# ethz-tb/orcAI

Hardware: AMD Instinct MI355X
Metric: audio_seconds_per_s (higher is better)
Workload: dtype f32; 1 GPU; orcai-V1 predict, 1 h synthetic recording @48 kHz, 1833 snippets; parallelism=independent recordings x1

## Files before the change

### include/orcai_hip.h

```cpp
#ifndef ORCAI_HIP_H
#define ORCAI_HIP_H

#include <stddef.h>
#include <stdint.h>

#ifdef __cplusplus
extern "C" {
#endif

#define ORCAI_E_BADARG (-1)
#define ORCAI_E_UNSUPPORTED (-2)

const char* orcai_version(void);


size_t orcai_frontend_workspace_bytes(void);

int orcai_frontend_reset(void* workspace, void* stream);

int orcai_pcm_decode(const void* frames, int64_t n_frames, int channels, int channel, int format, float* out, void* stream);

int orcai_pcm_decode_planar(const void* frames, int64_t n_frames, int channels, int format, float* out, int64_t stride, void* stream);

int orcai_resample_polyphase(const float* x, int64_t n_in, float* out, int64_t n_out, int L, int M, const float* table, int ntaps, void* stream);
// ... 107 lines not shown

int orcai_sepconv_route(int half, int Cin, int Cout, int H, int W, int out_layout, int extras);

int orcai_entry_windows(int windows_per_wave);

int orcai_entry_tile(int waves);

int orcai_conv0_bn_relu(const float* in, int64_t snippet_stride, int B, int H, int W, int ksize, const float* w, const float* scale,
                        const float* shift, float* out, void* stream);

int orcai_conv0_sepconv(const float* in, int64_t snippet_stride, int B, int H, int W, const float* w0, const float* scale0, const float* shift0,
                        const float* dw, const float* pw, const float* scale, const float* shift, int Cout, int relu_out, float* out, float* prev_sub,
                        void* stream);

int orcai_sepconv_bn(const float* in, int B, int Cin, int H, int W, int ksize, int relu_in, const float* dw, const float* pw, const float* scale,
                     const float* shift, int Cout, int relu_out, int out_layout, float* out, void* stream);

int orcai_pool_res_add(const float* s, const float* prev, int B, int C, int Cp, int H, int W, int ksize, const float* wr, const float* br,
                       float* out, int xpooled, void* stream);
int orcai_pool_res_add_scatter(const float* s, const float* prev, int B, int C, int Cp, int H, int W, int ksize, const float* wr, const float* br,
                               float* out, int xpooled, int Hd, int nsnip, int period, int base, int img_step, int r_lo, int r_hi, int keep_lo,
                               int keep_hi, void* stream);
#define ORCAI_ROW_FAMILIES 4
typedef struct {
  float* out;
  int Hd, period, offset, count, keep_lo, keep_hi;
} orcai_row_family;
int orcai_pool_res_add_scatter_families(const float* s, const float* prev, int B, int C, int Cp, int H, int W, int ksize, const float* wr,
                                        const float* br, int xpooled, int base, int img_step, int r_lo, int r_hi, const orcai_row_family* fams,
                                        int nfam, void* stream);
int orcai_sepconv_pool_res(const float* in, const float* prev, int B, int Cin, int C, int Cp, int H, int W, int ksize, int relu_in, const float* dw, const float* pw,
                           const float* scale, const float* shift, int relu_out, const float* wr, const float* br, float* out, int prev_compact, void* stream);
int orcai_pool_fused(int nt);
int orcai_pool_vertical(int on);

int orcai_gemm_bias_act(const float* A, const float* Bm, const float* bias, const float* scale, const float* shift, float* C, int64_t M, int N,
                        int K, int act, void* stream);

int orcai_lstm_recurrent(const float* xz, const float* Uw, int B, int T, int units, float* out, void* stream);

int orcai_dense_sigmoid(const float* x, const float* w, const float* bias, int64_t M, int K, int N, float* out, void* stream);

int orcai_overlap_average(const float* pred, int n, int P, int L, int step, int64_t S, double* agg, double* cnt, void* stream);

int orcai_overlap_average_ragged(const float* pred, int P, int L, int step, const int64_t* table, int R, int64_t S_total, double* agg, double* cnt,
                                 void* stream);

int orcai_extract_labels(const double* agg, const double* cnt, int L, const int64_t* table, int R, int64_t S_total, double threshold,
                         const int* label_rank, const double* limits, double frame_seconds, int tpo, int* runs, int64_t capacity, int64_t* offsets,
                         void* workspace, size_t workspace_bytes, void* stream);
size_t orcai_extract_labels_workspace_bytes(int L, int R, int64_t S_total);

int orcai_extract_labels_per_label(const double* agg, const double* cnt, int L, const int64_t* table, int R, int64_t S_total, const double* thresholds,
                                   const int* label_rank, const double* limits, double frame_seconds, int tpo, int* runs, int64_t capacity,
                                   int64_t* offsets, void* workspace, size_t workspace_bytes, void* stream);

int orcai_extract_labels_refined(const double* agg, const double* cnt, int L, const int64_t* table, int R, int64_t S_total, const double* thresholds,
                                 const double* high_thresholds, const int* gap_rows, const int* label_rank, const double* limits, double frame_seconds,
                                 int tpo, int* runs, int64_t capacity, int64_t* offsets, void* workspace, size_t workspace_bytes, void* stream);
size_t orcai_extract_labels_refined_workspace_bytes(int L, int R, int64_t S_total);

int orcai_interval_scores(const double* agg, int L, const int64_t* table, int R, int64_t S_total, const int* runs, const int64_t* offsets,
                          int64_t capacity, void* scores, void* eager, int64_t eager_runs, void* workspace, size_t workspace_bytes, void* stream);
size_t orcai_interval_scores_workspace_bytes(int L, int R, int64_t S_total);

int orcai_test_counts(const float* p, const float* y, int64_t M, int L, float mask_value, int64_t* conf, int64_t* mis, void* stream);
// ... 248 lines not shown
```

### orcai_amd/_native.py

```python

from __future__ import annotations

import ctypes as C
from pathlib import Path

LIB_PATH = Path(__file__).resolve().parent / "liborcai_hip.so"

_lib = None

c_i64 = C.c_int64
c_f32p = C.c_void_p

class UnpackDesc(C.Structure):

    _fields_ = [("src", C.c_void_p), ("ld_src", C.c_int), ("col_off", C.c_int), ("rows", C.c_int), ("G", C.c_void_p), ("W", C.c_void_p), ("l2g", C.c_float)]


class RowFamily(C.Structure):

    _fields_ = [("out", C.c_void_p), ("Hd", C.c_int), ("period", C.c_int), ("offset", C.c_int), ("count", C.c_int), ("keep_lo", C.c_int), ("keep_hi", C.c_int)]


_SIGNATURES = {
    "orcai_version": (C.c_char_p, []),
# ... 38 lines not shown
    "orcai_adam_step": (C.c_int, [C.c_void_p, C.c_void_p, C.c_void_p, C.c_void_p, c_i64, C.c_float, C.c_float, C.c_float, C.c_float, C.c_int, C.c_float, C.c_void_p]),
    "orcai_lstm_split": (C.c_int, [C.c_int]),
    "orcai_lstm_train_fwd": (C.c_int, [C.c_void_p, C.c_void_p, C.c_int, C.c_int, C.c_int, C.c_void_p, C.c_void_p, C.c_void_p, C.c_void_p]),
    "orcai_h_lstm_train_fwd": (C.c_int, [C.c_void_p, C.c_void_p, C.c_int, C.c_int, C.c_int, C.c_void_p, C.c_void_p, C.c_void_p, C.c_void_p]),
    "orcai_lstm_bwd": (C.c_int, [C.c_void_p, C.c_void_p, C.c_void_p, C.c_void_p, C.c_int, C.c_int, C.c_int, C.c_void_p, C.c_void_p]),
    "orcai_h_lstm_bwd": (C.c_int, [C.c_void_p, C.c_void_p, C.c_void_p, C.c_void_p, C.c_int, C.c_int, C.c_int, C.c_void_p, C.c_void_p]),
    "orcai_lstm_hprev": (C.c_int, [C.c_void_p, C.c_int, C.c_int, C.c_int, C.c_void_p, C.c_void_p]),
    "orcai_conv0_affine": (C.c_int, [C.c_void_p, c_i64, C.c_int, C.c_int, C.c_int, C.c_int, C.c_void_p, C.c_void_p, C.c_void_p, C.c_int, C.c_void_p, C.c_void_p]),
    "orcai_gather_snippets": (C.c_int, [C.c_void_p, C.c_void_p, C.c_int, C.c_int, C.c_int, C.c_void_p, C.c_void_p]),
    "orcai_downsample_labels": (C.c_int, [C.c_void_p, C.c_void_p] + [C.c_int] * 4 + [C.c_void_p, C.c_void_p]),
    "orcai_freq_mean_bwd": (C.c_int, [C.c_void_p, C.c_int64, C.c_int, C.c_int, C.c_void_p, C.c_void_p]),
    "orcai_conv1d_bwd": (C.c_int, [C.c_void_p] * 3 + [C.c_int] * 5 + [C.c_void_p] * 3),
    "orcai_bn_bwd_pointwise": (C.c_int, [C.c_void_p, C.c_void_p] + [C.c_int] * 5 + [C.c_void_p] * 4 + [C.c_float, C.c_int, C.c_void_p, C.c_int] + [C.c_void_p] * 3 + [C.c_int] + [C.c_void_p] * 3),
    "orcai_pw_wgrad_tiles": (C.c_int, [C.c_int]),
    "orcai_bn_bwd_pointwise_wgrad": (C.c_int, [C.c_void_p] * 3 + [C.c_int] * 5 + [C.c_void_p] * 4 + [C.c_float, C.c_int, C.c_void_p, C.c_int] + [C.c_void_p] * 3 + [C.c_int] + [C.c_void_p] * 3 + [c_i64, C.c_void_p]),
    "orcai_h_bn_bwd_pointwise_wgrad": (C.c_int, [C.c_void_p] * 3 + [C.c_int] * 5 + [C.c_void_p] * 4 + [C.c_float, C.c_int, C.c_void_p, C.c_int] + [C.c_void_p] * 3 + [C.c_int] + [C.c_void_p] * 3 + [c_i64, C.c_void_p]),
    "orcai_pool_res_add_bn": (C.c_int, [C.c_void_p, C.c_void_p] + [C.c_int] * 6 + [C.c_void_p] * 3 + [C.c_int] + [C.c_void_p] * 4 + [C.c_float, C.c_void_p]),
    "orcai_pool_bwd_bn": (C.c_int, [C.c_void_p, C.c_void_p] + [C.c_int] * 5 + [C.c_void_p] * 4 + [C.c_float, C.c_void_p, C.c_void_p]),
    "orcai_pool_bwd_bn_bias": (C.c_int, [C.c_void_p, C.c_void_p] + [C.c_int] * 5 + [C.c_void_p] * 4 + [C.c_float] + [C.c_void_p] * 4),
    "orcai_h_pool_bwd_bn_bias": (C.c_int, [C.c_void_p, C.c_void_p] + [C.c_int] * 5 + [C.c_void_p] * 4 + [C.c_float] + [C.c_void_p] * 4),
    "orcai_conv0_bn_bwd": (C.c_int, [C.c_void_p, C.c_int64, C.c_void_p, C.c_void_p] + [C.c_int] * 4 + [C.c_void_p] * 4 + [C.c_float] + [C.c_void_p] * 5),
    "orcai_conv0_stats": (C.c_int, [C.c_void_p, C.c_int64] + [C.c_int] * 4 + [C.c_void_p] * 5),
    "orcai_conv0_affine_bn": (C.c_int, [C.c_void_p, C.c_int64] + [C.c_int] * 4 + [C.c_void_p] * 7 + [C.c_float, C.c_int, C.c_void_p, C.c_void_p]),
    "orcai_conv0_bn_bwd_x": (C.c_int, [C.c_void_p, C.c_int64, C.c_void_p] + [C.c_int] * 4 + [C.c_void_p] * 6 + [C.c_float] + [C.c_void_p] * 5 + [c_i64, C.c_void_p]),
    "orcai_pack_weights": (C.c_int, [C.c_void_p, C.c_void_p, C.c_int, C.c_void_p, C.c_void_p]),
    "orcai_freq_mean": (C.c_int, [C.c_void_p, C.c_int64, C.c_int, C.c_int, C.c_void_p, C.c_void_p]),
    "orcai_conv1d_sigmoid": (C.c_int, [C.c_void_p] * 3 + [C.c_int] * 5 + [C.c_void_p, C.c_void_p]),
    "orcai_sepconv_planes": (C.c_int, [C.c_void_p] + [C.c_int] * 7 + [C.c_void_p] * 4 + [C.c_int] * 5 + [C.c_void_p, C.c_void_p]),
    "orcai_sepconv_planes_u": (C.c_int, [C.c_void_p] + [C.c_int] * 7 + [C.c_void_p] * 4 + [C.c_int] * 5 + [C.c_void_p, C.c_void_p, C.c_void_p]),
    "orcai_sepconv_planes_stats": (C.c_int, [C.c_void_p] + [C.c_int] * 5 + [C.c_void_p] * 4 + [C.c_int] + [C.c_void_p] * 4),
    "orcai_dw_wgrad_march": (C.c_int, [C.c_int]),
    "orcai_pool_vertical": (C.c_int, [C.c_int]),
    "orcai_pool_fused": (C.c_int, [C.c_int]),
    "orcai_sepconv_pool_res": (C.c_int, [C.c_void_p] * 2 + [C.c_int] * 8 + [C.c_void_p] * 4 + [C.c_int] + [C.c_void_p] * 3 + [C.c_int, C.c_void_p]),
    "orcai_dw_bwd_fused": (C.c_int, [C.c_void_p, C.c_void_p] + [C.c_int] * 5 + [C.c_void_p] * 3 + [C.c_int] + [C.c_void_p] * 4 + [C.c_float, C.c_int, C.c_void_p, C.c_void_p]),
    "orcai_dw_bwd_fused_conv0": (C.c_int, [C.c_void_p, C.c_int64, C.c_void_p] + [C.c_int] * 3 + [C.c_void_p] * 9 + [C.c_float, C.c_void_p, C.c_void_p, C.c_void_p]),
    "orcai_conv0_bn_bwd_x_ready": (C.c_int, [C.c_void_p, C.c_int64, C.c_void_p] + [C.c_int] * 4 + [C.c_void_p] * 6 + [C.c_float] + [C.c_void_p] * 5 + [c_i64, C.c_void_p]),
    "orcai_conv0_bn_bwd_dx": (C.c_int, [C.c_void_p, C.c_int64, C.c_void_p] + [C.c_int] * 4 + [C.c_void_p] * 6 + [C.c_float] + [C.c_void_p] * 3),
    "orcai_conv0_stats_march": (C.c_int, [C.c_void_p, C.c_int64] + [C.c_int] * 3 + [C.c_void_p] * 5),
    "orcai_conv0_march": (C.c_int, [C.c_int]),
    "orcai_h_dw_bwd_fused": (C.c_int, [C.c_void_p, C.c_void_p] + [C.c_int] * 5 + [C.c_void_p] * 3 + [C.c_int] + [C.c_void_p] * 4 + [C.c_float, C.c_int, C.c_void_p, C.c_void_p]),
    "orcai_h_dw_bwd_fused_res": (C.c_int, [C.c_void_p, C.c_void_p] + [C.c_int] * 4 + [C.c_void_p] * 7 + [C.c_float, C.c_int, C.c_void_p, C.c_void_p, C.c_void_p]),
    "orcai_h_conv0_bn_bwd_ready": (C.c_int, [C.c_void_p, C.c_int64, C.c_void_p, C.c_void_p] + [C.c_int] * 4 + [C.c_void_p] * 4 + [C.c_float] + [C.c_void_p] * 5),
    "orcai_dw_wgrad_bn": (C.c_int, [C.c_void_p, C.c_void_p] + [C.c_int] * 4 + [C.c_void_p] * 4 + [C.c_float, C.c_void_p, C.c_void_p]),
    "orcai_sepconv_planes_stats_bn": (C.c_int, [C.c_void_p] + [C.c_int] * 4 + [C.c_void_p] * 4 + [C.c_float] + [C.c_void_p] * 4 + [C.c_int] + [C.c_void_p] * 4),
    "orcai_sepconv_planes_epi": (C.c_int, [C.c_void_p] + [C.c_int] * 4 + [C.c_void_p] * 4 + [C.c_int, C.c_void_p, C.c_int] + [C.c_void_p] * 5 + [C.c_float, C.c_int, C.c_void_p, C.c_void_p]),
    "orcai_bn_finish_sharded": (C.c_int, [C.c_void_p] + [C.c_int] * 4 + [C.c_void_p] * 3),
    "orcai_h_sepconv_stats": (C.c_int, [C.c_void_p] + [C.c_int] * 5 + [C.c_void_p] * 4 + [C.c_int] + [C.c_void_p] * 4),
    "orcai_h_sepconv_stats_bn": (C.c_int, [C.c_void_p] + [C.c_int] * 4 + [C.c_void_p] * 4 + [C.c_float] + [C.c_void_p] * 4 + [C.c_int] + [C.c_void_p] * 4),
    "orcai_h_bn_finish_sharded": (C.c_int, [C.c_void_p] + [C.c_int] * 4 + [C.c_void_p] * 3),
    "orcai_bn_planes_stats": (C.c_int, [C.c_void_p] + [C.c_int] * 5 + [C.c_void_p] * 4),
    "orcai_bn_planes_apply": (C.c_int, [C.c_void_p] + [C.c_int] * 5 + [C.c_void_p] * 4 + [C.c_float, C.c_int, C.c_void_p, C.c_void_p]),
    "orcai_bn_planes_bwd": (C.c_int, [C.c_void_p, C.c_void_p] + [C.c_int] * 5 + [C.c_void_p] * 4 + [C.c_float, C.c_int] + [C.c_void_p] * 5),
    "orcai_planes_sum": (C.c_int, [C.c_void_p] + [C.c_int] * 5 + [C.c_void_p, C.c_void_p, C.c_int, C.c_void_p]),
    "orcai_pool_bwd": (C.c_int, [C.c_void_p, C.c_void_p] + [C.c_int] * 5 + [C.c_void_p, C.c_void_p]),
    "orcai_outer_reduce": (C.c_int, [C.c_void_p, C.c_int, C.c_void_p] + [C.c_int] * 8 + [C.c_void_p, C.c_void_p, C.c_int64, C.c_void_p]),
    "orcai_dw_wgrad": (C.c_int, [C.c_void_p, C.c_void_p] + [C.c_int] * 7 + [C.c_void_p, C.c_void_p]),
    "orcai_conv0_wgrad": (C.c_int, [C.c_void_p, c_i64, C.c_void_p] + [C.c_int] * 4 + [C.c_void_p, C.c_void_p]),
    "orcai_feat_to_planes": (C.c_int, [C.c_void_p] + [C.c_int] * 5 + [C.c_void_p, C.c_void_p]),
    "orcai_planes_relu_bwd": (C.c_int, [C.c_void_p, C.c_void_p, c_i64, C.c_void_p, C.c_void_p]),
    "orcai_resample_polyphase": (C.c_int, [C.c_void_p, c_i64, C.c_void_p, c_i64, C.c_int, C.c_int, C.c_void_p, C.c_int, C.c_void_p]),
    "orcai_resample_polyphase_bwd": (C.c_int, [C.c_void_p, c_i64, C.c_void_p, c_i64, C.c_int, C.c_int, C.c_void_p, C.c_int, C.c_void_p]),
    "orcai_h_conv0_affine": (C.c_int, [C.c_void_p, c_i64, C.c_int, C.c_int, C.c_int, C.c_int, C.c_void_p, C.c_void_p, C.c_void_p, C.c_int, C.c_void_p, C.c_void_p]),
    "orcai_h_conv0_affine_bn": (C.c_int, [C.c_void_p, c_i64, C.c_int, C.c_int, C.c_int, C.c_int, C.c_void_p, C.c_void_p, C.c_void_p, C.c_void_p, C.c_void_p, C.c_void_p, C.c_void_p, C.c_float, C.c_void_p, C.c_void_p, C.c_void_p]),
    "orcai_h_sepconv": (C.c_int, [C.c_void_p] + [C.c_int] * 7 + [C.c_void_p] * 4 + [C.c_int] * 5 + [C.c_void_p, C.c_void_p, C.c_void_p]),
    "orcai_h_pool_res_add": (C.c_int, [C.c_void_p, C.c_void_p] + [C.c_int] * 6 + [C.c_void_p] * 3 + [C.c_int] + [C.c_void_p] * 4 + [C.c_float, C.c_void_p]),
# ... 159 lines not shown
```

### orcai_amd/csrc/lds_optin.h

```cpp
#pragma once
#include <hip/hip_runtime.h>

namespace orcai_lds {
constexpr int MAXDEV = 64;
template <auto Kernel>
hipError_t ensure_dynamic_lds(size_t bytes) {
  static size_t granted[MAXDEV] = {};
  int dev = 0;
  hipError_t e = hipGetDevice(&dev);
  if (e == hipSuccess && (dev < 0 || dev >= MAXDEV)) e = hipErrorInvalidDevice;
  if (e != hipSuccess || bytes <= granted[dev]) return e;
  e = hipFuncSetAttribute((const void*)Kernel, hipFuncAttributeMaxDynamicSharedMemorySize, (int)bytes);
  if (e == hipSuccess) granted[dev] = bytes;
  return e;
}
}
```

### orcai_amd/csrc/model_fwd.hip

```cpp
#include <hip/hip_runtime.h>
#include <type_traits>

#include <cstdint>

#include "lds_dma.h"
#include "orcai_hip.h"
#include "sep_route.h"
#include "zero_fill.h"

__attribute__((visibility("hidden"))) int lstm_wide_fwd_launch(const float* xz, const float* Uw, int B, int T, int units, float* out, float* gates, float* cstate, void* stream);

int g_orcai_lstm_split = 1;

namespace {

typedef float f32x4 __attribute__((ext_vector_type(4)));

__device__ __forceinline__ f32x4 mfma16(float a, float b, f32x4 c) { return __builtin_amdgcn_mfma_f32_16x16x4f32(a, b, c, 0, 0, 0); }


__device__ __forceinline__ void xcd_remap(int& bx, int& by) {
  const unsigned nbx = gridDim.x, total = nbx * gridDim.y;
  const unsigned L = blockIdx.y * nbx + blockIdx.x;
  const unsigned k = L & 7u, q = total >> 3, r = total & 7u;
  const unsigned Lp = k * q + (k < r ? k : r) + (L >> 3);
  by = (int)(Lp / nbx);
  bx = (int)(Lp - (unsigned)by * nbx);
}

template <int KS>
__global__ __launch_bounds__(256) void conv0_kernel(const float* __restrict__ in, int64_t snippet_stride, int H, int W, int WP,
                                                     const float* __restrict__ w , const float* __restrict__ scale,
                                                     const float* __restrict__ shift, float* __restrict__ out , int relu,
                                                     const float* __restrict__ bn_mean = nullptr, const float* __restrict__ bn_var = nullptr,
                                                     const float* __restrict__ bn_gamma = nullptr, const float* __restrict__ bn_beta = nullptr, float bn_eps = 0.0f) {
  constexpr int TH = 8, TW = 32, R = KS / 2, HH = TH + KS - 1, HW = TW + KS - 1, HP_ = HW + 1;
  __shared__ float halo[HH][HP_];
  __shared__ float bn2_s[2][16];
// ... 806 lines not shown
  }
  if (STATS) {
#pragma unroll
    for (int j = 0; j < 16; ++j) {
      float a = st[j];
      a += __uint_as_float(__builtin_amdgcn_update_dpp(0u, __float_as_uint(a), 0x111 , 0xf, 0xf, true));
      a += __uint_as_float(__builtin_amdgcn_update_dpp(0u, __float_as_uint(a), 0x112 , 0xf, 0xf, true));
      a += __uint_as_float(__builtin_amdgcn_update_dpp(0u, __float_as_uint(a), 0x114 , 0xf, 0xf, true));
      a += __uint_as_float(__builtin_amdgcn_update_dpp(0u, __float_as_uint(a), 0x118 , 0xf, 0xf, true));
      st[j] = a;
    }
    if (lj == 15) {
#pragma unroll
      for (int j = 0; j < 16; j += 4) *reinterpret_cast<float4*>(&stat_s[wave][lk][j]) = make_float4(st[j], st[j + 1], st[j + 2], st[j + 3]);
    }
    __syncthreads();
    if (wave == 0) {
      const int g = lane >> 4, j = lane & 15;
      float tot = 0.0f;
#pragma unroll
      for (int w2 = 0; w2 < TR; ++w2) tot += stat_s[w2][g][j];
      const int cq = ((j >> 2) & 1) * 4 + g;
      if (cq < CQo) atomicAdd(&shards[(((bx + b * 7) & 31) * CQo + cq) * 8 + (j >> 3) * 4 + (j & 3)], (double)tot);
    }
  }
}

template <int CQ, bool RELU>
__global__ __launch_bounds__(512, 6) void sepconv_pool_march_kernel(const float* __restrict__ in , int Cin, int H, int W, int WP,
                                                                   const float* __restrict__ dw , const float* __restrict__ pw ,
                                                                   const float* __restrict__ scale, const float* __restrict__ shift, int Cout, int relu_out,
                                                                   const float* __restrict__ prev, int Cp, int prev_compact, const float* __restrict__ wr ,
                                                                   const float* __restrict__ br, float* __restrict__ out , int Ho, int Wo, int WPo,
                                                                   int nstrip, int NT) {
  constexpr int KK = 9, R = 1, lo = 2, VAL = 60, TR = 8, MT = 2, NPX = VAL / 2, XROW = 8 * NPX * 4;
  constexpr int SLOT = (TR + 2) * 256;
  __shared__ __attribute__((aligned(16))) float lds_f[2 * SLOT + 7 * XROW];
  __shared__ float pw_s[CQ * 4 * 16 * MT];
  __shared__ float sc_s[MT * 16], sh_s[MT * 16];
  __shared__ float wr_s[16 * MT * 16];
  static_assert(2 * XROW <= (TR + 2) * 256, "two exchange rows alias one input slot");
  const int lane = threadIdx.x & 63, wave = __builtin_amdgcn_readfirstlane(threadIdx.x >> 6);
  int bx, b;
  xcd_remap(bx, b);
  const int seg = bx / nstrip, strip = bx - seg * nstrip;
  const int NPS = 4 * NT - 1;
  const int p0 = seg * NPS, pend = (p0 + NPS < Ho) ? p0 + NPS : Ho;
  const int rb = 2 * p0, c0 = strip * VAL;
  const int ntile = (2 * (pend - p0) + 1 + TR - 1) / TR;
  const int lk = lane >> 4, lj = lane & 15;
  const int plane = (H + 2 * R) * WP;
  const int CQo = (Cout + 3) >> 2, CQp = (Cp + 3) >> 2;
  constexpr int CQr = CQ;
  const char* src = reinterpret_cast<const char*>(in) + (int64_t)b * CQr * plane * 16;
  const uint32_t lds0 = (uint32_t)(uintptr_t)&lds_f[0];
  const bool two = wave < 2;

  int64_t plane16 = (int64_t)plane * 16;
  auto issue = [&](int t, int cq, int sl, int lane) {
    const int r0 = rb + t * TR;
    auto goff = [&](int j) {
      const int i = (r0 + j) * WP + c0 - lo + lane;
      return (uint32_t)(i < 0 ? 0 : (i >= plane ? plane - 1 : i)) * 16u;
    };
    const char* base = src + (int64_t)cq * plane16;
    const uint32_t slot = lds0 + (uint32_t)(sl * (TR + 2) * 1024);
    glds16(base + goff(wave), slot + (uint32_t)wave * 1024u);
    if (two) glds16(base + goff(TR + (wave & 1)), slot + (uint32_t)(TR + wave) * 1024u);
  };
  issue(0, 0, 0, lane);

  for (int i = threadIdx.x; i < CQ * 4 * 16 * MT; i += 64 * TR) {
    const int m = i % MT, lj_ = (i / MT) % 16, ci = i / (16 * MT), co = m * 16 + lj_;
    pw_s[i] = (ci < Cin && co < Cout) ? pw[ci * Cout + co] : 0.0f;
  }
  if (threadIdx.x < MT * 16) {
    const int co = threadIdx.x;
    sc_s[co] = co < Cout ? scale[co] : 0.0f;
    sh_s[co] = co < Cout ? shift[co] : 0.0f;
  }
  {
// ... 523 lines not shown
      }                                                                                                         \
    }                                                                                                           \
  }
  if (AHEAD) {
    ORCAI_POOL_LOAD_TILE(0, va)
    ORCAI_POOL_LOAD_TILE(1, vb)
    ORCAI_POOL_REDUCE_TILE(0, va)
    ORCAI_POOL_LOAD_TILE(2, va)
    ORCAI_POOL_REDUCE_TILE(1, vb)
    ORCAI_POOL_LOAD_TILE(3, vb)
    ORCAI_POOL_REDUCE_TILE(2, va)
    ORCAI_POOL_REDUCE_TILE(3, vb)
  } else {
    ORCAI_POOL_LOAD_TILE(0, va)
    ORCAI_POOL_REDUCE_TILE(0, va)
    ORCAI_POOL_LOAD_TILE(1, va)
    ORCAI_POOL_REDUCE_TILE(1, va)
    ORCAI_POOL_LOAD_TILE(2, va)
    ORCAI_POOL_REDUCE_TILE(2, va)
    ORCAI_POOL_LOAD_TILE(3, va)
    ORCAI_POOL_REDUCE_TILE(3, va)
  }
#undef ORCAI_POOL_LOAD_TILE
#undef ORCAI_POOL_REDUCE_TILE
}

struct RowFamily {
  float* out;
  int Hd, period, offset, count, keep_lo, keep_hi;
};
constexpr int kRowFamilies = ORCAI_ROW_FAMILIES;
struct RowMap {
  int base, img_step, r_lo, r_hi, nfam;
  RowFamily f[kRowFamilies];
};

template <int MT, bool VERT = false, bool SCATTER = false>
__global__ __launch_bounds__(256, MT <= 2 ? 4 : 2) void pool_res_add_x_kernel(const float* __restrict__ s , const float* __restrict__ prev, int C, int Cp, int H,
                                                              int W, int WP, int R, int Ho, int Wo, int WPo, int pad_top, const float* __restrict__ wr ,
                                                              const float* __restrict__ br, float* __restrict__ out , int prev_compact,
                                                              int tasks, uint32_t magic_WPo, int ntc = 0 ,
                                                              RowMap rm = RowMap{} ) {
  const int lane = threadIdx.x & 63;
  int bx, b;
  xcd_remap(bx, b);
  const int task = bx * 4 + (threadIdx.x >> 6);
  if (task >= tasks) return;
  const int lk = lane >> 4, lj = lane & 15;
  const int CQ = (C + 3) >> 2, CQp = (Cp + 3) >> 2;
  const int plane = prev_compact ? Ho * Wo : (H + 2 * R) * WP, plane_o = (Ho + 2 * R) * WPo;
  const int WPx = (Wo + 3) & ~3;
  const int qbase = R * WPo + task * 64;
  const int vrg = VERT ? task / ntc : 0, vct = VERT ? task - vrg * ntc : 0;

  constexpr int NROW = VERT ? 9 : 12;
  int soff[NROW], oidx[4];
#pragma unroll
  for (int t = 0; t < 4; ++t) {
    int i, jj, flat;
    if (VERT) {
      i = vrg * 4 + t;
      jj = vct * 16 + lj;
      flat = (i + R) * WPo + jj;
    } else {
      flat = qbase + 16 * t + lj;
      const int row = (int)__umulhi((uint32_t)flat, magic_WPo);
      jj = flat - row * WPo;
      i = row - R;
    }
    const bool valid = jj < Wo && i < Ho;
    oidx[t] = valid ? flat : -1;
#pragma unroll
    for (int dy = 0; dy < 3; ++dy) {
      if (VERT && t > 0 && dy == 0) continue;
      int y = 2 * i - pad_top + dy;
      y = y < 0 ? 0 : (y >= H ? H - 1 : y);
      const int jc = jj < Wo ? jj : Wo - 1;
      soff[VERT ? 2 * t + dy : 3 * t + dy] = VERT ? y * WPx + jc : (valid ? y * WPx + jj : 0);
    }
  }
  const char* sbase = reinterpret_cast<const char*>(reinterpret_cast<const float4*>(s) + (int64_t)b * CQ * H * WPx);
  uint32_t qoff[MT];
#pragma unroll
  for (int m = 0; m < MT; ++m) {
    const int oq = m * 4 + lk;
    qoff[m] = (uint32_t)((oq < CQ ? oq : 0) * H * WPx);
  }
  float4 v[NROW][MT];
  auto load_tile = [&](int t) {
#pragma unroll
    for (int m = 0; m < MT; ++m)
#pragma unroll
      for (int dy = 0; dy < 3; ++dy) {
        if (VERT && t > 0 && dy == 0) continue;
        const int e = VERT ? 2 * t + dy : 3 * t + dy;
        v[e][m] = *reinterpret_cast<const float4*>(sbase + (qoff[m] + (uint32_t)soff[e]) * 16u);
      }
  };
  float br_r[MT][4];
#pragma unroll
  for (int m = 0; m < MT; ++m)
#pragma unroll
    for (int r = 0; r < 4; ++r) {
      const int co = m * 16 + lk * 4 + r;
      const float bv = br[co < C ? co : 0];
      br_r[m][r] = co < C ? bv : 0.0f;
    }
  constexpr int DEPTH = MT <= 2 ? 2 : 1;
  load_tile(0);
  if (DEPTH > 1) load_tile(1);
  __builtin_amdgcn_sched_barrier(0);

  int pj, pi;
  if (VERT) {
    pi = vrg * 4 + lk;
    pj = vct * 16 + lj;
  } else {
    const int q = qbase + lane;
    const int prow = (int)__umulhi((uint32_t)q, magic_WPo);
    pj = q - prow * WPo;
    pi = prow - R;
  }
  const bool pvalid = pj < Wo && pi < Ho;
  const int srcpix = pvalid ? (prev_compact ? pi * Wo + pj : (2 * pi + R) * WP + 2 * pj) : 0;
  const float4* pp = reinterpret_cast<const float4*>(prev) + (int64_t)b * CQp * plane + srcpix;
  f32x4 acc[MT][4];
#pragma unroll
  for (int m = 0; m < MT; ++m)
#pragma unroll
    for (int t = 0; t < 4; ++t) acc[m][t] = (f32x4){0.f, 0.f, 0.f, 0.f};
  float4 nxt = pp[0];
  for (int cq = 0; cq < CQp; ++cq) {
    const float4 cur = nxt;
    if (cq + 1 < CQp) nxt = pp[(int64_t)(cq + 1) * plane];
    float afrag[MT];
#pragma unroll
    for (int m = 0; m < MT; ++m) {
      const int ci = cq * 4 + lk, co = m * 16 + lj;
      const bool ok = ci < Cp && co < C;
      const float av = wr[ok ? ci * C + co : 0];
      afrag[m] = ok ? av : 0.0f;
    }
    float d[4] = {cur.x, cur.y, cur.z, cur.w};
    swap32(d[0], d[2]);
    swap32(d[1], d[3]);
    swap16(d[0], d[1]);
    swap16(d[2], d[3]);
#pragma unroll
// ... 859 lines not shown
  if ((xpooled & 1) && tot_w / 2 != 0) return ORCAI_E_UNSUPPORTED;
  if (xpooled & ~3) return ORCAI_E_BADARG;
  if (bn_mean && (xpooled || !bn_var || !bn_gamma || !bn_beta)) return ORCAI_E_BADARG;
  const int WP = orcai_padded_width(W, ksize), WPo = orcai_padded_width(Wo, ksize), R = ksize / 2;
  const int tasks = (Ho * WPo + 63) / 64;
  dim3 grid((tasks + 3) / 4, B);
  hipStream_t st = (hipStream_t)stream;
  const uint32_t mg = magic_for(WPo);
  const int ntc = (Wo + 15) / 16, vtasks = ntc * ((Ho + 3) / 4);
  const bool vert = g_pool_vert && Wo >= 40;
  dim3 vgrid((vtasks + 3) / 4, B);
#define ORCAI_POOL_LAUNCH(MT)                                                                                                                        \
  if ((xpooled & 1) && !bn_mean && (int64_t)((C + 3) / 4) * H * (((Wo + 3) & ~3)) < (1ll << 28)) {                                                                   \
    if (vert)                                                                                                                                        \
      hipLaunchKernelGGL((pool_res_add_x_kernel<MT, true>), vgrid, dim3(256), 0, st, s, prev, C, Cp, H, W, WP, R, Ho, Wo, WPo, tot_h / 2, wr, br, out,            \
                         (xpooled >> 1) & 1, vtasks, mg, ntc);                                                                                       \
    else                                                                                                                                             \
      hipLaunchKernelGGL((pool_res_add_x_kernel<MT, false>), grid, dim3(256), 0, st, s, prev, C, Cp, H, W, WP, R, Ho, Wo, WPo, tot_h / 2, wr, br, out,            \
                         (xpooled >> 1) & 1, tasks, mg, 0);                                                                                          \
  } else                                                                                                                                               \
    hipLaunchKernelGGL(pool_res_add_kernel<MT>, grid, dim3(256), 0, st, s, prev, C, Cp, H, W, WP, R, Ho, Wo, WPo, tot_h / 2, tot_w / 2, wr, br, out, xpooled, tasks, mg, bn_mean, bn_var, bn_gamma, bn_beta, bn_eps)
  switch ((C + 15) / 16) {
    case 1: ORCAI_POOL_LAUNCH(1); break;
    case 2: ORCAI_POOL_LAUNCH(2); break;
    case 3: ORCAI_POOL_LAUNCH(3); break;
    case 4: ORCAI_POOL_LAUNCH(4); break;
    default: return ORCAI_E_UNSUPPORTED;
  }
#undef ORCAI_POOL_LAUNCH
  return (int)hipGetLastError();
}

int g_pool_fused_nt = 8;

int orcai_pool_fused(int nt) {
  const int prev = g_pool_fused_nt;
  if (nt >= 0) g_pool_fused_nt = nt > 64 ? 64 : nt;
  return prev;
}

int orcai_sepconv_pool_res(const float* in, const float* prev, int B, int Cin, int C, int Cp, int H, int W, int ksize, int relu_in, const float* dw, const float* pw,
                           const float* scale, const float* shift, int relu_out, const float* wr, const float* br, float* out, int prev_compact, void* stream) {
  if (!in || !prev || !dw || !pw || !scale || !shift || !wr || !br || !out || B <= 0 || Cin <= 0 || C <= 0 || Cp <= 0 || H <= 0 || W <= 0) return ORCAI_E_BADARG;
  const int nstrip = orcai_route::wide_strips(W, 60), CQ = (Cin + 3) / 4, WP = orcai_padded_width(W, 3);
  if (g_pool_fused_nt <= 0 || g_tile_mode != 1 || ksize != 3 || (C + 15) / 16 != 2 || CQ < 5 || CQ > 8 || Cp > 16 || (H & 1) || !nstrip ||
      ((uintptr_t)in & 15) || ((uintptr_t)prev & 15) || ((uintptr_t)out & 15) || B > 65535 || (int64_t)8 * (H + 2) * WP >= (1ll << 27))
    return ORCAI_E_UNSUPPORTED;
  const int Ho = H / 2, Wo = (W + 1) / 2, WPo = orcai_padded_width(Wo, 3);
  const int NT = g_pool_fused_nt, nseg = (Ho + 4 * NT - 2) / (4 * NT - 1);
  dim3 grid(nstrip * nseg, B);
  hipStream_t st = (hipStream_t)stream;
#define ORCAI_PM_LAUNCH(CQT, RELU)                                                                                                                          \
  hipLaunchKernelGGL((sepconv_pool_march_kernel<CQT, RELU>), grid, dim3(512), 0, st, in, Cin, H, W, WP, dw, pw, scale, shift, C, relu_out, prev, Cp, prev_compact ? 1 : 0, \
                     wr, br, out, Ho, Wo, WPo, nstrip, NT)
  switch (CQ) {
    case 5: if (relu_in) ORCAI_PM_LAUNCH(5, true); else ORCAI_PM_LAUNCH(5, false); break;
    case 6: if (relu_in) ORCAI_PM_LAUNCH(6, true); else ORCAI_PM_LAUNCH(6, false); break;
    case 7: if (relu_in) ORCAI_PM_LAUNCH(7, true); else ORCAI_PM_LAUNCH(7, false); break;
    case 8: if (relu_in) ORCAI_PM_LAUNCH(8, true); else ORCAI_PM_LAUNCH(8, false); break;
    default: return ORCAI_E_UNSUPPORTED;
  }
#undef ORCAI_PM_LAUNCH
  return (int)hipGetLastError();
}

int orcai_pool_vertical(int on) {
  const int prev = g_pool_vert;
  if (on >= 0) g_pool_vert = on ? 1 : 0;
  return prev;
}

int orcai_pool_res_add(const float* s, const float* prev, int B, int C, int Cp, int H, int W, int ksize, const float* wr, const float* br, float* out,
                       int xpooled, void* stream) {
  return orcai_pool_res_add_bn(s, prev, B, C, Cp, H, W, ksize, wr, br, out, xpooled, nullptr, nullptr, nullptr, nullptr, 0.0f, stream);
}

static int pool_res_scatter_launch(const float* s, const float* prev, int B, int C, int Cp, int H, int W, int ksize, const float* wr, const float* br,
                                   int xpooled, RowMap rm, void* stream) {
  const int Ho = (H + 1) / 2, Wo = (W + 1) / 2;
  const int tot_w = (Wo - 1) * 2 + 2 - W;
  if (!(xpooled & 1) || (tot_w > 0 ? tot_w : 0) / 2 != 0 || (C + 15) / 16 > 4 || (int64_t)((C + 3) / 4) * H * ((Wo + 3) & ~3) >= (1ll << 28))
    return ORCAI_E_UNSUPPORTED;
  if ((int64_t)rm.base + (int64_t)(B - 1) * rm.img_step + Ho >= (1ll << 31)) return ORCAI_E_UNSUPPORTED;
  int tot_h = (Ho - 1) * 2 + 3 - H;
  if (tot_h < 0) tot_h = 0;
  const int WP = orcai_padded_width(W, ksize), WPo = orcai_padded_width(Wo, ksize), R = ksize / 2;
  rm.r_lo = rm.r_lo < 0 ? 0 : rm.r_lo;
  rm.r_hi = rm.r_hi > Ho ? Ho : rm.r_hi;
  const int tasks = (Ho * WPo + 63) / 64;
  const int ntc = (Wo + 15) / 16, vtasks = ntc * ((Ho + 3) / 4);
  const bool vert = g_pool_vert && Wo >= 40;
  const dim3 grid((tasks + 3) / 4, B), vgrid((vtasks + 3) / 4, B);
  hipStream_t st = (hipStream_t)stream;
  const uint32_t mg = magic_for(WPo);
  const int compact = (xpooled >> 1) & 1;
  float* out = rm.f[0].out;
#define ORCAI_POOL_SCATTER(MT)                                                                                                                                  \
  if (vert)                                                                                                                                                      \
    hipLaunchKernelGGL((pool_res_add_x_kernel<MT, true, true>), vgrid, dim3(256), 0, st, s, prev, C, Cp, H, W, WP, R, Ho, Wo, WPo, tot_h / 2, wr, br, out, compact, \
                       vtasks, mg, ntc, rm);                                                                                                                     \
  else                                                                                                                                                           \
    hipLaunchKernelGGL((pool_res_add_x_kernel<MT, false, true>), grid, dim3(256), 0, st, s, prev, C, Cp, H, W, WP, R, Ho, Wo, WPo, tot_h / 2, wr, br, out, compact, \
                       tasks, mg, 0, rm)
  switch ((C + 15) / 16) {
    case 1: ORCAI_POOL_SCATTER(1); break;
    case 2: ORCAI_POOL_SCATTER(2); break;
    case 3: ORCAI_POOL_SCATTER(3); break;
    case 4: ORCAI_POOL_SCATTER(4); break;
  }
#undef ORCAI_POOL_SCATTER
  return (int)hipGetLastError();
}

int orcai_pool_res_add_scatter(const float* s, const float* prev, int B, int C, int Cp, int H, int W, int ksize, const float* wr, const float* br, float* out,
                               int xpooled, int Hd, int nsnip, int period, int base, int img_step, int r_lo, int r_hi, int keep_lo, int keep_hi,
                               void* stream) {
  if (!s || !prev || !wr || !br || !out || B <= 0 || C <= 0 || Cp <= 0 || H <= 0 || W <= 0 || nsnip <= 0 || period <= 0) return ORCAI_E_BADARG;
  if (xpooled & ~3) return ORCAI_E_BADARG;
  if (keep_lo < 0 || keep_hi > Hd || keep_lo >= keep_hi || Hd != 2 * period || base < 0 || img_step < 0) return ORCAI_E_BADARG;
  RowMap rm{};
  rm.base = base;
  rm.img_step = img_step;
  rm.r_lo = r_lo;
  rm.r_hi = r_hi;
// ... 103 lines not shown
```

Baseline: 152,700 audio-s/s.

## Taper fused sepconv-pool march segments to fill the final wave of workgroups

Replaces the fixed 2D grid of uniform row segments with a 1D plan. Bulk segments fill whole waves of resident workgroups, and the leftover rows are split into progressively shorter segments (tapering) so the last partial wave is better balanced. Occupancy is queried per kernel to size the waves, and the in-kernel decode also interleaves bulk indices in groups of 8, replacing the earlier xcd_remap. This adds decode arithmetic per workgroup and extra halo overhead from the shorter segments.

Result: no change. 153,000 audio-s/s, median of 6 (+0.2%).

```diff
diff --git a/include/orcai_hip.h b/include/orcai_hip.h
--- a/include/orcai_hip.h
+++ b/include/orcai_hip.h
@@ -163,6 +163,9 @@
 int orcai_sepconv_pool_res(const float* in, const float* prev, int B, int Cin, int C, int Cp, int H, int W, int ksize, int relu_in, const float* dw, const float* pw,
                            const float* scale, const float* shift, int relu_out, const float* wr, const float* br, float* out, int prev_compact, void* stream);
 int orcai_pool_fused(int nt);
+int orcai_pool_fused_slots(int n);
+int orcai_pool_fused_plan(int Ho, int S, int nt, int slots, int* out);
+int orcai_pool_fused_plan_decode(int Ho, int S, int nstrip, int nt, int slots, int first, int count, int* out);
 int orcai_pool_vertical(int on);
 
 int orcai_gemm_bias_act(const float* A, const float* Bm, const float* bias, const float* scale, const float* shift, float* C, int64_t M, int N,
diff --git a/orcai_amd/_native.py b/orcai_amd/_native.py
--- a/orcai_amd/_native.py
+++ b/orcai_amd/_native.py
@@ -94,6 +94,9 @@
     "orcai_dw_wgrad_march": (C.c_int, [C.c_int]),
     "orcai_pool_vertical": (C.c_int, [C.c_int]),
     "orcai_pool_fused": (C.c_int, [C.c_int]),
+    "orcai_pool_fused_slots": (C.c_int, [C.c_int]),
+    "orcai_pool_fused_plan": (C.c_int, [C.c_int] * 4 + [C.c_void_p]),
+    "orcai_pool_fused_plan_decode": (C.c_int, [C.c_int] * 7 + [C.c_void_p]),
     "orcai_sepconv_pool_res": (C.c_int, [C.c_void_p] * 2 + [C.c_int] * 8 + [C.c_void_p] * 4 + [C.c_int] + [C.c_void_p] * 3 + [C.c_int, C.c_void_p]),
     "orcai_dw_bwd_fused": (C.c_int, [C.c_void_p, C.c_void_p] + [C.c_int] * 5 + [C.c_void_p] * 3 + [C.c_int] + [C.c_void_p] * 4 + [C.c_float, C.c_int, C.c_void_p, C.c_void_p]),
     "orcai_dw_bwd_fused_conv0": (C.c_int, [C.c_void_p, C.c_int64, C.c_void_p] + [C.c_int] * 3 + [C.c_void_p] * 9 + [C.c_float, C.c_void_p, C.c_void_p, C.c_void_p]),
diff --git a/orcai_amd/csrc/lds_optin.h b/orcai_amd/csrc/lds_optin.h
--- a/orcai_amd/csrc/lds_optin.h
+++ b/orcai_amd/csrc/lds_optin.h
@@ -14,4 +14,20 @@
   if (e == hipSuccess) granted[dev] = bytes;
   return e;
 }
+
+template <auto Kernel>
+int resident_workgroups(int threads) {
+  static int slots[MAXDEV] = {};
+  static bool known[MAXDEV] = {};
+  int dev = 0;
+  if (hipGetDevice(&dev) != hipSuccess || dev < 0 || dev >= MAXDEV) return 0;
+  if (!known[dev]) {
+    int cus = 0, per_cu = 0;
+    if (hipDeviceGetAttribute(&cus, hipDeviceAttributeMultiprocessorCount, dev) == hipSuccess &&
+        hipOccupancyMaxActiveBlocksPerMultiprocessor(&per_cu, (const void*)Kernel, threads, 0) == hipSuccess && cus > 0 && per_cu > 0)
+      slots[dev] = cus * per_cu;
+    known[dev] = true;
+  }
+  return slots[dev];
 }
+}
diff --git a/orcai_amd/csrc/march_plan.h b/orcai_amd/csrc/march_plan.h
--- /dev/null
+++ b/orcai_amd/csrc/march_plan.h
@@ -0,0 +1,86 @@
+#pragma once
+#include <cstdint>
+
+#if defined(__HIPCC__)
+#define ORCAI_MARCH_HD __host__ __device__
+#else
+#define ORCAI_MARCH_HD
+#endif
+
+namespace orcai_march {
+constexpr int kMaxTaper = 5;
+
+struct Plan {
+  int NT, nb, n_bulk;
+  int S;
+  int len[kMaxTaper];
+  int cnt[kMaxTaper];
+};
+
+struct Segment {
+  int image, strip, p0, ntile;
+};
+
+inline int64_t workgroups(const Plan& p) {
+  int64_t per = p.nb;
+  for (int e = 0; e < kMaxTaper; ++e) per += p.cnt[e];
+  return per * p.S;
+}
+
+inline Plan make_plan(int Ho, int S, int NT, int slots) {
+  Plan p{};
+  const int NPS = 4 * NT - 1;
+  const int nseg = (Ho + NPS - 1) / NPS;
+  p.NT = NT, p.S = S, p.nb = nseg;
+  const int64_t G = (int64_t)S * nseg;
+  p.n_bulk = (int)G;
+  if (slots <= 0 || G <= slots || NT < 4 || nseg < 2) return p;
+  const int64_t R = G / slots, f = G - R * slots;
+  if (f == 0 || f * 20 >= (int64_t)slots * 19) return p;
+  const int nb = (int)(R * slots / S);
+  int left = Ho - nb * NPS, e = 0;
+  for (int l = NT / 2; l >= 2 && left > 0; l /= 2) {
+    const int rows = 4 * l - 1;
+    const int c = l / 2 < 2 ? (left + rows - 1) / rows : (left / 2) / rows;
+    if (!c) continue;
+    p.len[e] = l, p.cnt[e] = c, ++e;
+    left -= c * rows;
+  }
+  p.nb = nb, p.n_bulk = (int)((int64_t)S * nb);
+  return p;
+}
+
+ORCAI_MARCH_HD inline Segment decode(const Plan& p, int nstrip, unsigned L) {
+  Segment s;
+  const unsigned nbulk = (unsigned)p.n_bulk;
+  if (L < nbulk) {
+    const unsigned k = L & 7u, q = nbulk >> 3, r = nbulk & 7u;
+    const unsigned Lp = k * q + (k < r ? k : r) + (L >> 3);
+    const unsigned per = (unsigned)(nstrip * p.nb);
+    const unsigned b = Lp / per, bx = Lp - b * per;
+    const unsigned seg = bx / (unsigned)nstrip;
+    s.image = (int)b, s.strip = (int)(bx - seg * (unsigned)nstrip), s.p0 = (int)seg * (4 * p.NT - 1), s.ntile = p.NT;
+    return s;
+  }
+  unsigned rem = L - nbulk;
+  int p0 = p.nb * (4 * p.NT - 1), n = 0;
+  unsigned si = 0;
+  bool found = false;
+#pragma unroll
+  for (int e = 0; e < kMaxTaper; ++e) {
+    const int rows = 4 * p.len[e] - 1;
+    const unsigned wgs = (unsigned)p.cnt[e] * (unsigned)p.S;
+    if (!found) {
+      if (rem < wgs) {
+        const unsigned k = rem / (unsigned)p.S;
+        found = true, n = p.len[e], si = rem - k * (unsigned)p.S, p0 += (int)k * rows;
+      } else {
+        rem -= wgs, p0 += p.cnt[e] * rows;
+      }
+    }
+  }
+  const unsigned b = si / (unsigned)nstrip;
+  s.image = (int)b, s.strip = (int)(si - b * (unsigned)nstrip), s.p0 = p0, s.ntile = n;
+  return s;
+}
+}
diff --git a/orcai_amd/csrc/model_fwd.hip b/orcai_amd/csrc/model_fwd.hip
--- a/orcai_amd/csrc/model_fwd.hip
+++ b/orcai_amd/csrc/model_fwd.hip
@@ -4,6 +4,8 @@
 #include <cstdint>
 
 #include "lds_dma.h"
+#include "lds_optin.h"
+#include "march_plan.h"
 #include "orcai_hip.h"
 #include "sep_route.h"
 #include "zero_fill.h"
@@ -876,7 +878,7 @@
                                                                    const float* __restrict__ scale, const float* __restrict__ shift, int Cout, int relu_out,
                                                                    const float* __restrict__ prev, int Cp, int prev_compact, const float* __restrict__ wr ,
                                                                    const float* __restrict__ br, float* __restrict__ out , int Ho, int Wo, int WPo,
-                                                                   int nstrip, int NT) {
+                                                                   int nstrip, orcai_march::Plan mp) {
   constexpr int KK = 9, R = 1, lo = 2, VAL = 60, TR = 8, MT = 2, NPX = VAL / 2, XROW = 8 * NPX * 4;
   constexpr int SLOT = (TR + 2) * 256;
   __shared__ __attribute__((aligned(16))) float lds_f[2 * SLOT + 7 * XROW];
@@ -885,12 +887,11 @@
   __shared__ float wr_s[16 * MT * 16];
   static_assert(2 * XROW <= (TR + 2) * 256, "two exchange rows alias one input slot");
   const int lane = threadIdx.x & 63, wave = __builtin_amdgcn_readfirstlane(threadIdx.x >> 6);
-  int bx, b;
-  xcd_remap(bx, b);
-  const int seg = bx / nstrip, strip = bx - seg * nstrip;
-  const int NPS = 4 * NT - 1;
-  const int p0 = seg * NPS, pend = (p0 + NPS < Ho) ? p0 + NPS : Ho;
-  const int rb = 2 * p0, c0 = strip * VAL;
+  const orcai_march::Segment sg = orcai_march::decode(mp, nstrip, blockIdx.x);
+  const int b = sg.image;
+  const int NPS = 4 * sg.ntile - 1;
+  const int p0 = sg.p0, pend = (p0 + NPS < Ho) ? p0 + NPS : Ho;
+  const int rb = 2 * p0, c0 = sg.strip * VAL;
   const int ntile = (2 * (pend - p0) + 1 + TR - 1) / TR;
   const int lk = lane >> 4, lj = lane & 15;
   const int plane = (H + 2 * R) * WP;
@@ -2487,11 +2488,41 @@
 }
 
 int g_pool_fused_nt = 8;
+int g_pool_fused_slots = 0;
 
 int orcai_pool_fused(int nt) {
   const int prev = g_pool_fused_nt;
   if (nt >= 0) g_pool_fused_nt = nt > 64 ? 64 : nt;
   return prev;
+}
+
+int orcai_pool_fused_slots(int n) {
+  const int prev = g_pool_fused_slots;
+  if (n >= 0) g_pool_fused_slots = n;
+  return prev;
+}
+
+int orcai_pool_fused_plan(int Ho, int S, int nt, int slots, int* out) {
+  if (Ho <= 0 || S <= 0 || nt <= 0 || nt > 64 || !out) return ORCAI_E_BADARG;
+  if ((int64_t)S * ((Ho + 4 * nt - 2) / (4 * nt - 1)) >= (1ll << 31)) return ORCAI_E_UNSUPPORTED;
+  const orcai_march::Plan p = orcai_march::make_plan(Ho, S, nt, slots);
+  const int64_t wgs = orcai_march::workgroups(p);
+  if (wgs >= (1ll << 31)) return ORCAI_E_UNSUPPORTED;
+  out[0] = p.nb, out[1] = p.n_bulk;
+  for (int e = 0; e < orcai_march::kMaxTaper; ++e) out[2 + e] = p.len[e], out[2 + orcai_march::kMaxTaper + e] = p.cnt[e];
+  return (int)wgs;
+}
+
+int orcai_pool_fused_plan_decode(int Ho, int S, int nstrip, int nt, int slots, int first, int count, int* out) {
+  if (Ho <= 0 || S <= 0 || nstrip <= 0 || S % nstrip || nt <= 0 || nt > 64 || first < 0 || count < 0 || !out) return ORCAI_E_BADARG;
+  if ((int64_t)S * ((Ho + 4 * nt - 2) / (4 * nt - 1)) >= (1ll << 31)) return ORCAI_E_UNSUPPORTED;
+  const orcai_march::Plan p = orcai_march::make_plan(Ho, S, nt, slots);
+  if ((int64_t)first + count > orcai_march::workgroups(p)) return ORCAI_E_BADARG;
+  for (int i = 0; i < count; ++i) {
+    const orcai_march::Segment s = orcai_march::decode(p, nstrip, (unsigned)(first + i));
+    out[4 * i] = s.image, out[4 * i + 1] = s.strip, out[4 * i + 2] = s.p0, out[4 * i + 3] = s.ntile;
+  }
+  return 0;
 }
 
 int orcai_sepconv_pool_res(const float* in, const float* prev, int B, int Cin, int C, int Cp, int H, int W, int ksize, int relu_in, const float* dw, const float* pw,
@@ -2502,12 +2533,17 @@
       ((uintptr_t)in & 15) || ((uintptr_t)prev & 15) || ((uintptr_t)out & 15) || B > 65535 || (int64_t)8 * (H + 2) * WP >= (1ll << 27))
     return ORCAI_E_UNSUPPORTED;
   const int Ho = H / 2, Wo = (W + 1) / 2, WPo = orcai_padded_width(Wo, 3);
-  const int NT = g_pool_fused_nt, nseg = (Ho + 4 * NT - 2) / (4 * NT - 1);
-  dim3 grid(nstrip * nseg, B);
+  const int NT = g_pool_fused_nt;
+  if ((int64_t)nstrip * B * ((Ho + 4 * NT - 2) / (4 * NT - 1)) >= (1ll << 31)) return ORCAI_E_UNSUPPORTED;
   hipStream_t st = (hipStream_t)stream;
 #define ORCAI_PM_LAUNCH(CQT, RELU)                                                                                                                          \
-  hipLaunchKernelGGL((sepconv_pool_march_kernel<CQT, RELU>), grid, dim3(512), 0, st, in, Cin, H, W, WP, dw, pw, scale, shift, C, relu_out, prev, Cp, prev_compact ? 1 : 0, \
-                     wr, br, out, Ho, Wo, WPo, nstrip, NT)
+  do {                                                                                                                                                      \
+    const int slots = g_pool_fused_slots ? g_pool_fused_slots : orcai_lds::resident_workgroups<sepconv_pool_march_kernel<CQT, RELU>>(512);                        \
+    const orcai_march::Plan mp = orcai_march::make_plan(Ho, nstrip * B, NT, slots);                                                                        \
+    if (orcai_march::workgroups(mp) >= (1ll << 31)) return ORCAI_E_UNSUPPORTED;                                                                             \
+    hipLaunchKernelGGL((sepconv_pool_march_kernel<CQT, RELU>), dim3((unsigned)orcai_march::workgroups(mp)), dim3(512), 0, st, in, Cin, H, W, WP, dw, pw, scale, shift, C, \
+                       relu_out, prev, Cp, prev_compact ? 1 : 0, wr, br, out, Ho, Wo, WPo, nstrip, mp);                                                     \
+  } while (0)
   switch (CQ) {
     case 5: if (relu_in) ORCAI_PM_LAUNCH(5, true); else ORCAI_PM_LAUNCH(5, false); break;
     case 6: if (relu_in) ORCAI_PM_LAUNCH(6, true); else ORCAI_PM_LAUNCH(6, false); break;
```

## Skip pooled-residual scatter tasks whose output rows are all discarded

Applied to the files above, without the earlier changes.

Adds a rowmap_keeps helper that checks whether any output row in a range survives the row-family keep windows. The host binary-searches the first and last kept rows across the batch and shrinks the launch grid to that span via a new org offset. Inside the kernel, each wave exits early when none of its rows are kept. This cuts wasted compute and memory traffic on rows that overlapping snippet stitching throws away. In exchange it adds host-side search cost and more complex indexing, which could go wrong at image edges.

After: 151,300 audio-s/s before, 151,900 audio-s/s after, median of 6. Within noise of the previous version (+0.4%).

```diff
diff --git a/orcai_amd/csrc/model_fwd.hip b/orcai_amd/csrc/model_fwd.hip
--- a/orcai_amd/csrc/model_fwd.hip
+++ b/orcai_amd/csrc/model_fwd.hip
@@ -1480,8 +1480,29 @@
 constexpr int kRowFamilies = ORCAI_ROW_FAMILIES;
 struct RowMap {
   int base, img_step, r_lo, r_hi, nfam;
+  int org;
   RowFamily f[kRowFamilies];
 };
+
+__host__ __device__ __forceinline__ bool rowmap_keeps(const RowMap& rm, int b, int ra, int rb) {
+  const int origin = rm.base + b * rm.img_step;
+  const int lo = origin == 0 ? 0 : rm.r_lo;
+  ra = ra < lo ? lo : ra;
+  rb = rb > rm.r_hi ? rm.r_hi : rb;
+  if (ra >= rb) return false;
+  bool any = false;
+#pragma unroll
+  for (int fi = 0; fi < kRowFamilies; ++fi) {
+    if (fi >= rm.nfam) break;
+    const RowFamily& fm = rm.f[fi];
+    const int rel = origin + rb - 1 - fm.offset - fm.keep_lo;
+    if (rel < 0) continue;
+    int j = rel / fm.period;
+    j = j < fm.count ? j : fm.count - 1;
+    any |= origin + ra - fm.offset - j * fm.period < fm.keep_hi;
+  }
+  return any;
+}
 
 template <int MT, bool VERT = false, bool SCATTER = false>
 __global__ __launch_bounds__(256, MT <= 2 ? 4 : 2) void pool_res_add_x_kernel(const float* __restrict__ s , const float* __restrict__ prev, int C, int Cp, int H,
@@ -1492,14 +1513,20 @@
   const int lane = threadIdx.x & 63;
   int bx, b;
   xcd_remap(bx, b);
-  const int task = bx * 4 + (threadIdx.x >> 6);
+  const int task = bx * 4 + (SCATTER ? __builtin_amdgcn_readfirstlane((int)(threadIdx.x >> 6)) : (int)(threadIdx.x >> 6));
   if (task >= tasks) return;
   const int lk = lane >> 4, lj = lane & 15;
   const int CQ = (C + 3) >> 2, CQp = (Cp + 3) >> 2;
   const int plane = prev_compact ? Ho * Wo : (H + 2 * R) * WP, plane_o = (Ho + 2 * R) * WPo;
   const int WPx = (Wo + 3) & ~3;
-  const int qbase = R * WPo + task * 64;
+  const int qbase = R * WPo + (SCATTER && !VERT ? rm.org : 0) + task * 64;
   const int vrg = VERT ? task / ntc : 0, vct = VERT ? task - vrg * ntc : 0;
+  const int vrow = (SCATTER ? rm.org : 0) + vrg * 4;
+  if (SCATTER) {
+    const int ra = VERT ? vrow : (int)__umulhi((uint32_t)qbase, magic_WPo) - R;
+    const int rb = VERT ? vrow + 4 : (int)__umulhi((uint32_t)qbase + 63u, magic_WPo) - R + 1;
+    if (!rowmap_keeps(rm, b, ra, rb < Ho ? rb : Ho)) return;
+  }
 
   constexpr int NROW = VERT ? 9 : 12;
   int soff[NROW], oidx[4];
@@ -1507,7 +1534,7 @@
   for (int t = 0; t < 4; ++t) {
     int i, jj, flat;
     if (VERT) {
-      i = vrg * 4 + t;
+      i = vrow + t;
       jj = vct * 16 + lj;
       flat = (i + R) * WPo + jj;
     } else {
@@ -1561,7 +1588,7 @@
 
   int pj, pi;
   if (VERT) {
-    pi = vrg * 4 + lk;
+    pi = vrow + lk;
     pj = vct * 16 + lj;
   } else {
     const int q = qbase + lane;
@@ -2542,9 +2569,33 @@
   const int WP = orcai_padded_width(W, ksize), WPo = orcai_padded_width(Wo, ksize), R = ksize / 2;
   rm.r_lo = rm.r_lo < 0 ? 0 : rm.r_lo;
   rm.r_hi = rm.r_hi > Ho ? Ho : rm.r_hi;
-  const int tasks = (Ho * WPo + 63) / 64;
-  const int ntc = (Wo + 15) / 16, vtasks = ntc * ((Ho + 3) / 4);
+  int first = Ho, last = 0;
+  for (int b = 0; b < B; ++b) {
+    if (first > 0 && rowmap_keeps(rm, b, 0, first)) {
+      int lo = 0, hi = first;
+      while (hi - lo > 1) {
+        const int mid = lo + (hi - lo) / 2;
+        if (rowmap_keeps(rm, b, 0, mid)) hi = mid; else lo = mid;
+      }
+      first = hi - 1;
+    }
+    if (last < Ho && rowmap_keeps(rm, b, last, Ho)) {
+      int lo = last, hi = Ho;
+      while (hi - lo > 1) {
+        const int mid = lo + (hi - lo) / 2;
+        if (rowmap_keeps(rm, b, mid, Ho)) lo = mid; else hi = mid;
+      }
+      last = lo + 1;
+    }
+  }
+  if (first >= last) return (int)hipGetLastError();
   const bool vert = g_pool_vert && Wo >= 40;
+  const bool shortimg = Ho < 8;
+  const int row0 = shortimg ? first : first & ~3;
+  const int q0 = shortimg ? first * WPo : first * WPo / 64 * 64;
+  rm.org = vert ? row0 : q0;
+  const int tasks = (last * WPo - q0 + 63) / 64;
+  const int ntc = (Wo + 15) / 16, vtasks = ntc * ((last - row0 + 3) / 4);
   const dim3 grid((tasks + 3) / 4, B), vgrid((vtasks + 3) / 4, B);
   hipStream_t st = (hipStream_t)stream;
   const uint32_t mg = magic_for(WPo);
```
